# r-barnes/richdem

Hardware: AMD Instinct MI355X
Metric: Mcells/s Priority-Flood fill, 40k x 40k f32 DEM (higher is better)
Workload: dtype f32; 1 GPU; 40000x40000 float32 fractal value-noise DEM G(seed=3), FillDepressions<D8>, HBM-resident; cells=1600000000, basins=10332798, boruvka_rounds=9, pair_records=39443163, jump_passes=1, parallelism=1 GPU

## Files before the change

include/rdgpu.h:

```cpp
#ifndef RDGPU_H_
#define RDGPU_H_

#include <stdint.h>

#ifdef __cplusplus
extern "C" {
#endif

#define RDGPU_OK 0
#define RDGPU_ERR_HIP 1
#define RDGPU_ERR_ARG 2
#define RDGPU_ERR_UNSUPPORTED 3
#define RDGPU_ERR_CAPACITY 4

const char *rdgpu_last_error(void);
const char *rdgpu_version(void);
int rdgpu_device_count(int *count);
int rdgpu_set_device(int device_id);
int rdgpu_release_workspace(void);

int rdgpu_fill_u8(uint8_t *dem, int width, int height, int topology);
int rdgpu_fill_i16(int16_t *dem, int width, int height, int topology);
int rdgpu_fill_u16(uint16_t *dem, int width, int height, int topology);
int rdgpu_fill_i32(int32_t *dem, int width, int height, int topology);
// ... 124 lines not shown
  int rdgpu_watersheds_##SUF(T *dem, T nodata, int width, int height, int topology, int alter, int32_t *labels);      \
  int rdgpu_watersheds_dev_##SUF(T *d_dem, T nodata, int width, int height, int topology, int alter, int32_t *d_labels, void *hip_stream);
RDGPU_DECL_WS(u8, uint8_t)
RDGPU_DECL_WS(i16, int16_t)
RDGPU_DECL_WS(u16, uint16_t)
RDGPU_DECL_WS(i32, int32_t)
RDGPU_DECL_WS(u32, uint32_t)
RDGPU_DECL_WS(f32, float)
RDGPU_DECL_WS(i8, int8_t)
RDGPU_DECL_WS(f64, double)
RDGPU_DECL_WS(i64, int64_t)
RDGPU_DECL_WS(u64, uint64_t)
#undef RDGPU_DECL_WS

typedef struct rdgpu_fill_stats {
  uint64_t cells;
  uint64_t basins;
  uint32_t rounds;
  uint32_t jump_passes;
  uint64_t scan_tiles;
  uint32_t tile_cells;
  uint32_t edge_records;
  uint32_t host_syncs;
  uint32_t reserved;
} rdgpu_fill_stats;
int rdgpu_fill_get_stats(rdgpu_fill_stats *out);

typedef struct rdgpu_fill_shard rdgpu_fill_shard;
int rdgpu_fill_shard_begin_u8(uint8_t *d_rows, int width, int rows, int topology, int open_top, int open_bottom, void *hip_stream, rdgpu_fill_shard **out);
int rdgpu_fill_shard_begin_i16(int16_t *d_rows, int width, int rows, int topology, int open_top, int open_bottom, void *hip_stream, rdgpu_fill_shard **out);
int rdgpu_fill_shard_begin_u16(uint16_t *d_rows, int width, int rows, int topology, int open_top, int open_bottom, void *hip_stream, rdgpu_fill_shard **out);
int rdgpu_fill_shard_begin_i32(int32_t *d_rows, int width, int rows, int topology, int open_top, int open_bottom, void *hip_stream, rdgpu_fill_shard **out);
int rdgpu_fill_shard_begin_u32(uint32_t *d_rows, int width, int rows, int topology, int open_top, int open_bottom, void *hip_stream, rdgpu_fill_shard **out);
int rdgpu_fill_shard_begin_f32(float *d_rows, int width, int rows, int topology, int open_top, int open_bottom, void *hip_stream, rdgpu_fill_shard **out);
int rdgpu_fill_shard_begin_i8(int8_t *d_rows, int width, int rows, int topology, int open_top, int open_bottom, void *hip_stream, rdgpu_fill_shard **out);
int rdgpu_fill_shard_edge_count(rdgpu_fill_shard *shard, uint32_t *n_edges);
int rdgpu_fill_shard_export(rdgpu_fill_shard *shard, uint32_t *top_keys, uint32_t *bottom_keys, uint32_t *edges);
int rdgpu_fill_shard_finish(rdgpu_fill_shard *shard, const uint32_t *levels);
int rdgpu_fill_shard_free(rdgpu_fill_shard *shard);
int rdgpu_fill_graph_solve(int nshards, int width, int topology, const uint32_t *keys, const uint32_t *edges,
                           const uint64_t *edge_offsets, uint32_t *levels);
int rdgpu_fill_shard_export_dev(rdgpu_fill_shard *shard, uint32_t *d_keys, uint32_t *d_edges, uint32_t cap);
int rdgpu_fill_graph_solve_dev(int nshards, int width, int topology, const uint32_t *d_keys_all,
                               const uint32_t *d_edges_all, const uint32_t *d_counts, uint32_t cap,
                               uint32_t *d_levels_all, void *hip_stream);
int rdgpu_fill_shard_finish_dev(rdgpu_fill_shard *shard, const uint32_t *d_levels);
int rdgpu_fill_multi_u8(uint8_t *dem, int width, int height, int topology, const int *devices, int ndevices);
// ... 457 lines not shown
```

richdem_amd/_lib.py:

```python
from __future__ import annotations

import ctypes
import os
import subprocess

_HERE = os.path.dirname(os.path.abspath(__file__))
_LIB = None


class RdgpuError(RuntimeError):
    """Raised when a C-ABI call returns non-zero (mirrors the reference's std::runtime_error)."""


def lib_path() -> str:
    return os.environ.get("RDGPU_LIB") or os.path.join(_HERE, "librdgpu.so")


def build(force: bool = False) -> str:
    args = ["make", "-C", os.path.join(_HERE, "csrc"), "-j8"]
    if force:
        subprocess.check_call(args + ["clean"], stdout=subprocess.DEVNULL)
    subprocess.check_call(args, stdout=subprocess.DEVNULL)
    return lib_path()


class rdgpu_fill_stats(ctypes.Structure):
    _fields_ = [
        ("cells", ctypes.c_uint64),
        ("basins", ctypes.c_uint64),
        ("rounds", ctypes.c_uint32),
        ("jump_passes", ctypes.c_uint32),
        ("scan_tiles", ctypes.c_uint64),
        ("tile_cells", ctypes.c_uint32),
        ("edge_records", ctypes.c_uint32),
        ("host_syncs", ctypes.c_uint32),
        ("reserved", ctypes.c_uint32),
    ]


def lib() -> ctypes.CDLL:
    global _LIB
    if _LIB is None:
        p = lib_path()
        if not os.path.exists(p):
            raise RdgpuError(
                f"{p} is missing: the HIP extension is not built (run richdem_amd.build() / "
                "python -c 'import __graft_entry__ as g; g.build()').  There is no CPU fallback."
            )
        try:
            import torch
        except ImportError:
            pass
        L = ctypes.CDLL(p)
        L.rdgpu_last_error.restype = ctypes.c_char_p
        L.rdgpu_version.restype = ctypes.c_char_p
        L.rdgpu_profile_name.restype = ctypes.c_char_p
        _LIB = L
    return _LIB


def check(rc: int, what: str = "") -> None:
    if rc != 0:
        msg = lib().rdgpu_last_error().decode(errors="replace")
        err = RdgpuError(f"{what}: {msg} (code {rc})" if what else f"{msg} (code {rc})")
        err.code = rc
        raise err


def fill_stats() -> dict:
    st = rdgpu_fill_stats()
    check(lib().rdgpu_fill_get_stats(ctypes.byref(st)), "rdgpu_fill_get_stats")
    return {"cells": st.cells, "basins": st.basins, "rounds": st.rounds, "jump_passes": st.jump_passes,
            "scan_tiles": st.scan_tiles, "tile_cells": st.tile_cells, "edge_records": st.edge_records,
            "host_syncs": st.host_syncs}


def profile_enable(on: bool = True) -> None:
    lib().rdgpu_profile_enable(1 if on else 0)


def profile_collect() -> None:
    check(lib().rdgpu_profile_collect(), "rdgpu_profile_collect")


def profile_reset() -> None:
    check(lib().rdgpu_profile_reset(), "rdgpu_profile_reset")


def profile_totals() -> dict:
    L = lib()
    profile_collect()
    out = {}
    i = 0
    while True:
        nm = L.rdgpu_profile_name(i)
        if nm is None:
            break
# ... 7 lines not shown
```

richdem_amd/csrc/fill.hip:

```cpp
#include "common.hpp"
#include "fill_shared.hpp"

#include <algorithm>
#include <cstdlib>
#include <vector>

struct rdgpu_fill_shard;

namespace rdgpu {

constexpr int TW = 64;
constexpr int TH = 32;
constexpr int LW = TW + 2;
constexpr int LH = TH + 2;
constexpr uint32_t OUTP = 0xFFFFFFFFu;
constexpr uint32_t CLOSED = 0x80000000u;
constexpr uint32_t NO_TID = 0xFFFFFFFFu;

static thread_local rdgpu_fill_stats g_stats;

constexpr int DW = 64, DH = 64, DLW = DW + 2, DLH = DH + 2;
constexpr uint32_t LAB_PEND = 0x80000000u;
constexpr uint16_t LTERM_BASE = 0xF000u;

// ... 1694 lines not shown
  check_fill_args(dem, w, h, topology);
  const size_t bytes = (size_t)w * h * sizeof(T);
  T *d = Workspace::get().buf<T>("host.dem", (size_t)w * h);
  RD_HIP(hipMemcpy(d, dem, bytes, hipMemcpyHostToDevice));
  fill_max_dep_device<T>(d, w, h, topology, max_dep, nullptr);
  RD_HIP(hipStreamSynchronize(nullptr));
  RD_HIP(hipMemcpy(dem, d, bytes, hipMemcpyDeviceToHost));
}

constexpr int FSTRIPES = 32, FSTRIDE = 16;
struct FusedBuf {
  uint16_t *lab16;
  uint32_t *G;
  uint32_t *tile_base, *tile_count;
  unsigned long long *counters;
  uint32_t gcap, rcap, smask;
  uint32_t *overflow;
  uint32_t *edgeK = nullptr;
  uint16_t *edgeS = nullptr;
  uint16_t *edgeR = nullptr;
};

__global__ __launch_bounds__(64) void k_stripe_offsets(const unsigned long long *__restrict__ counters, uint32_t nstripes,
                                                       uint32_t *pitoff, uint32_t *out) {
  const uint32_t s = threadIdx.x;
  const unsigned long long c = s < nstripes ? counters[s * FSTRIDE] : 0ull;
  const uint32_t pits = (uint32_t)c, nodes = (uint32_t)(c >> 32);
  uint32_t incl = pits, tot = nodes, mx = nodes;
#pragma unroll
  for (int o = 1; o < 64; o <<= 1) {
    const uint32_t v = __shfl_up(incl, o, 64);
    if ((int)s >= o) incl += v;
    tot += __shfl_xor(tot, o, 64);
    mx = max(mx, (uint32_t)__shfl_xor(mx, o, 64));
  }
  if (s < nstripes) pitoff[s] = incl - pits;
  if (s == 63) { out[0] = incl; out[1] = tot; out[2] = mx; }
}

template <class T, int TOPO, bool VEC, bool OUTLETS = false, bool CUT = false>
__global__ __launch_bounds__(NTHR) void k_descent16(const T *__restrict__ z, FusedBuf fo, int w, int h,
                                                    uint32_t tilesX, uint32_t ntiles, const uint8_t *__restrict__ outlet = nullptr,
                                                    const uint8_t *__restrict__ skip = nullptr,
                                                    const uint32_t *__restrict__ tlist = nullptr, int open_top = 0,
                                                    int open_bottom = 0) {
  __shared__ uint32_t sk[DLH * DLW];
  constexpr int LPD = DW + 2;
  __shared__ uint16_t lp[DH * LPD];
  __shared__ uint32_t wtot[NTHR / 64];
  __shared__ uint32_t pbase, rbase, fits_s;
  const uint32_t t = (OUTLETS && tlist) ? tlist[blockIdx.x] : xcd_tile(blockIdx.x, ntiles);
  if (t >= ntiles) return;
  const int x0 = (int)(t % tilesX) * DW, y0 = (int)(t / tilesX) * DH;
  if (OUTLETS && skip && skip[t]) {
    if (threadIdx.x == 0) { fo.tile_base[t] = 0; fo.tile_count[t] = 1; }
    if (skip[t] == 1) {
      const int lx_ = threadIdx.x & (DW - 1), gx_ = x0 + lx_;
      for (int ly_ = threadIdx.x >> 6; ly_ < DH; ly_ += NTHR / 64)
        if (gx_ < w && y0 + ly_ < h) fo.lab16[(size_t)(y0 + ly_) * w + gx_] = 0;
    }
    return;
  }
  const bool inner = !OUTLETS && x0 >= 1 && y0 >= 1 && x0 + DW <= w - 1 && y0 + DH <= h - 1;
  {
    constexpr int NQ = DLH * (DW / 4), QPT = (NQ + NTHR - 1) / NTHR;
    Quad<T> zq[QPT];
    if (y0 >= 1 && y0 + DH < h && x0 + DW <= w) {
#pragma unroll
// ... 22 lines not shown
        const int gx = x0 + 4 * q, gy = y0 - 1 + ly;
        okq[r] = i < NQ && gy >= 0 && gy < h && gx < w;
        if (okq[r]) zq[r] = load_quad<T, VEC>(z + (size_t)gy * w, gx, w, T());
      }
#pragma unroll
      for (int r = 0; r < QPT; r++) keys_after_loads(zq[r]);
#pragma unroll
      for (int r = 0; r < QPT; r++) {
        const int i = threadIdx.x + r * NTHR;
        if (i >= NQ) continue;
        const int ly = i / (DW / 4), q = i - ly * (DW / 4);
        const int o = ly * DLW + 1 + 4 * q;
#pragma unroll
        for (int e = 0; e < 4; e++) sk[o + e] = (okq[r] && x0 + 4 * q + e < w) ? key32_fast<T>(zq[r].v[e]) : 0xFFFFFFFFu;
      }
    }
    for (int i = threadIdx.x; i < 2 * DLH; i += NTHR) {
      const int ly = i >> 1, lxh = (i & 1) ? DLW - 1 : 0;
      const int gx = x0 - 1 + lxh, gy = y0 - 1 + ly;
      uint32_t kk = 0xFFFFFFFFu;
      if (gx >= 0 && gx < w && gy >= 0 && gy < h) kk = key32_fast<T>(z[(size_t)gy * w + gx]);
      sk[ly * DLW + lxh] = kk;
    }
  }
  __syncthreads();
  const int wave_s = __builtin_amdgcn_readfirstlane((int)(threadIdx.x >> 6));
  const int lx = threadIdx.x & (DW - 1), ly0 = wave_s * (DH / 4);
  const int gx = x0 + lx;
  constexpr int RPT = DH / 4;
  static_assert(RPT == 16, "four code words of four bytes, 16-bit row masks");
  uint16_t *const slot16 = reinterpret_cast<uint16_t *>(sk);
  const uint32_t selfb0 = (uint32_t)((ly0 * LPD + lx) * 2);
  uint32_t p[RPT];
  uint32_t codes[RPT / 4] = {0, 0, 0, 0};
  uint32_t rootmask = 0, pitmask = 0, outmask = 0;
  {
    constexpr uint32_t WT0 = 0u | (1u << 16) | (1u << 24) | (1u << 27), WT1 = 2u | (2u << 16) | (1u << 25) | (1u << 27),
                       WT2 = 4u | (3u << 16) | (1u << 26) | (1u << 27);
    constexpr uint32_t WM0 = (uint32_t)(2 * LPD) | (4u << 16) | (1u << 24), WM2 = (uint32_t)(2 * LPD + 4) | (5u << 16) | (1u << 26);
    constexpr uint32_t BADD = (uint32_t)(4 * LPD) + (5u << 16) + ((1u << 29) - (1u << 27));
    const bool colin = gx < w, colborder = (gx == 0) | (gx == w - 1);
    const uint32_t cmcol = lx == 0 ? (1u << 24) : lx == DW - 1 ? (1u << 26) : 0u;
    uint32_t ta, tb, tc, tm, tW, ma, mb, mc, mm3, mW;
    auto triple = [&](int r, uint32_t &a, uint32_t &b, uint32_t &c, uint32_t &m, uint32_t &W) {
      a = sk[r * DLW + lx];
      b = sk[r * DLW + lx + 1];
      c = sk[r * DLW + lx + 2];
      if (TOPO == 8) {
        m = min(min(a, b), c);
        W = a == m ? WT0 : b == m ? WT1 : WT2;
      } else {
        m = b;
        W = WT1;
      }
    };
    triple(ly0, ta, tb, tc, tm, tW);
    triple(ly0 + 1, ma, mb, mc, mm3, mW);
// ... 9 lines not shown
      const uint32_t bk = min(min(tm, mm), bm);
      const bool isT = tm == bk, isM = mm == bk;
      const uint32_t wM = midfirst ? WM0 : WM2, wB = bW + BADD, wMB = isM ? wM : wB;
      const uint32_t W = isT ? tW : wMB;
      const bool drains = (bk < kc) | ((bk == kc) & (isT | (isM & midfirst)));
      uint32_t cm = cmcol;
      if (j == 0 && ly0 == 0) cm |= 1u << 27;
      if (j == RPT - 1 && ly0 == DH - RPT) cm |= 1u << 29;
      const bool outside = (W & cm) != 0u;
      const uint32_t self = selfb0 + (uint32_t)(j * LPD * 2);
      const bool incell = INNER || (colin & (gy < h));
      bool border = !INNER && (colborder | (gy == 0) | (gy == h - 1));
      bool stays = !drains;
      if (CUT && !INNER) {
        const bool cutrow = ((gy == 0) & (open_top != 0)) | ((gy == h - 1) & (open_bottom != 0));
        border = colborder | ((gy == 0) & !open_top) | ((gy == h - 1) & !open_bottom);
        stays |= cutrow;
      }
      if (OUTLETS) border |= incell && outlet[(size_t)gy * w + gx] != 0;
      const bool selfp = !incell | border | stays | outside;
      const uint32_t rel = selfp ? (uint32_t)(2 * LPD + 2) : (W & 0xFFFFu);
      p[j] = rel + (self - (uint32_t)(2 * LPD + 2));
      *reinterpret_cast<uint16_t *>(reinterpret_cast<char *>(lp) + self) = (uint16_t)p[j];
      const uint32_t cexit = (W >> 16) & 15u, cin = stays ? 0u : cexit;
      const uint32_t code = border ? 9u : cin;
      codes[j >> 2] |= code << (8 * (j & 3));
      bool root = incell & selfp;
      if (OUTLETS) {
        const bool outroot = root & border;
        outmask |= (outroot ? 1u : 0u) << j;
        root &= !outroot;
      }
      rootmask |= (root ? 1u : 0u) << j;
      pitmask |= ((root & !border & stays) ? 1u : 0u) << j;
      ta = ma; tb = mb; tc = mc; tm = mm3; tW = mW;
      ma = ba; mb = bb; mc = bc; mm3 = bm; mW = bW;
    }
    };
    if (inner) classify(std::true_type());
    else classify(std::false_type());
    (void)ta; (void)tb; (void)tc;
  }
  asm volatile("" : "+v"(rootmask), "+v"(pitmask), "+v"(outmask), "+v"(codes[0]), "+v"(codes[1]), "+v"(codes[2]), "+v"(codes[3]));
  if (fo.edgeK && threadIdx.x < 2 * DH) {
    const int side = threadIdx.x >> 6, lye = threadIdx.x & (DH - 1), lxe = side ? DW - 1 : 0;
    fo.edgeK[((size_t)t * 2 + side) * DH + lye] = sk[(lye + 1) * DLW + lxe + 1];
  }
  __syncthreads();
  {
    const char *const lpb = reinterpret_cast<const char *>(lp);
    uint32_t gact = (1u << (RPT / 4)) - 1u;
    constexpr int BLIND = 2;
    for (int it = 0; it < BLIND; it++) {
      asm volatile("" ::: "memory");
#pragma unroll
      for (int g = 0; g < RPT / 4; g++) {
        uint32_t qv[4], rv[4];
#pragma unroll
        for (int e = 0; e < 4; e++) { qv[e] = *reinterpret_cast<const uint16_t *>(lpb + p[4 * g + e]); asm("" : "+v"(qv[e])); }
#pragma unroll
        for (int e = 0; e < 4; e++) { rv[e] = *reinterpret_cast<const uint16_t *>(lpb + qv[e]); asm("" : "+v"(rv[e])); }
#pragma unroll
        for (int e = 0; e < 4; e++) {
          const int j = 4 * g + e;
          p[j] = rv[e];
          *reinterpret_cast<uint16_t *>(reinterpret_cast<char *>(lp) + selfb0 + (uint32_t)(j * LPD * 2)) = (uint16_t)rv[e];
        }
      }
    }
    for (int it = 0; gact != 0u && it < DW * DH; it++) {
      asm volatile("" ::: "memory");
// ... 18 lines not shown
    }
  }
  const uint32_t mine = ((uint32_t)__popc(rootmask) << 16) | (uint32_t)__popc(pitmask);
  uint32_t incl = mine;
#pragma unroll
  for (int o = 1; o < 64; o <<= 1) {
    const uint32_t v = __shfl_up(incl, o, 64);
    if ((threadIdx.x & 63) >= o) incl += v;
  }
  if ((threadIdx.x & 63) == 63) wtot[threadIdx.x >> 6] = incl;
  __syncthreads();
  if (threadIdx.x == 0) {
    const uint32_t nr = (wtot[0] >> 16) + (wtot[1] >> 16) + (wtot[2] >> 16) + (wtot[3] >> 16) + (OUTLETS ? 1u : 0u);
    const uint32_t np = (wtot[0] & 0xFFFFu) + (wtot[1] & 0xFFFFu) + (wtot[2] & 0xFFFFu) + (wtot[3] & 0xFFFFu);
    const uint32_t st = t & fo.smask;
    const unsigned long long old = atomicAdd(&fo.counters[st * FSTRIDE], ((unsigned long long)nr << 32) | np);
    const uint32_t rl = (uint32_t)(old >> 32);
    pbase = (uint32_t)old;
    rbase = st * fo.rcap + rl;
    fo.tile_base[t] = rbase;
    fo.tile_count[t] = nr;
    fits_s = (unsigned long long)rl + nr <= fo.rcap ? 1u : 0u;
    if (!fits_s) *fo.overflow = 1;
  }
  {
    uint32_t pre = incl - mine;
    for (int k = 0; k < wave_s; k++) pre += wtot[k];
    uint32_t slot = (pre >> 16) + (OUTLETS ? 1u : 0u);
    if (OUTLETS)
      for (uint32_t m = outmask; m; m &= m - 1)
        *reinterpret_cast<uint16_t *>(reinterpret_cast<char *>(slot16) + selfb0 + (uint32_t)((__ffs((int)m) - 1) * LPD * 2)) = 0;
    for (uint32_t m = rootmask; m; m &= m - 1) {
      const int j = __ffs((int)m) - 1;
      *reinterpret_cast<uint16_t *>(reinterpret_cast<char *>(slot16) + selfb0 + (uint32_t)(j * LPD * 2)) = (uint16_t)slot;
      slot++;
    }
  }
  __syncthreads();
  const uint32_t nodes0 = rbase;
  if (fits_s != 0) {
    uint32_t pre = incl - mine;
    for (int k = 0; k < wave_s; k++) pre += wtot[k];
    uint32_t slot = (pre >> 16) + (OUTLETS ? 1u : 0u), pit = pbase + (pre & 0xFFFFu);
    if (OUTLETS && threadIdx.x == 0) fo.G[nodes0] = OUTP;
    for (uint32_t m = rootmask; m; m &= m - 1) {
      const int j = __ffs((int)m) - 1;
      const int ly = ly0 + j;
      const uint32_t cw = j < 8 ? (j < 4 ? codes[0] : codes[1]) : (j < 12 ? codes[2] : codes[3]);
      const int code = (int)(cw >> (8 * (j & 3)) & 15u);
      const int n = code <= 4 ? code - 1 : code;
      const int nr = n >= 6 ? 2 : n >= 3 ? 1 : 0, nc = n - 3 * nr;
      const uint32_t pend = LAB_PEND | ((uint32_t)(y0 + ly + nr - 1) * (uint32_t)w + (uint32_t)(x0 + lx + nc - 1));
      const uint32_t word = code == 0 ? pit++ : code == 9 ? OUTP : pend;
      fo.G[nodes0 + slot] = word;
      slot++;
    }
  }
  {
    const char *const sl = reinterpret_cast<const char *>(slot16);
    if (inner) {
#pragma unroll
      for (int j = 0; j < RPT; j++) {
        const int gy = y0 + ly0 + j;
        fo.lab16[(size_t)gy * w + gx] = *reinterpret_cast<const uint16_t *>(sl + p[j]);
      }
    } else {
#pragma unroll
      for (int j = 0; j < RPT; j++) {
        const int gy = y0 + ly0 + j;
        const uint16_t rv = *reinterpret_cast<const uint16_t *>(sl + p[j]);
        if ((gx < w) & (gy < h)) fo.lab16[(size_t)gy * w + gx] = rv;
      }
    }
    if (fo.edgeS && threadIdx.x < 2 * DH) {
      const int side = threadIdx.x >> 6, lye = threadIdx.x & (DH - 1), lxe = side ? DW - 1 : 0;
      const uint16_t v = lp[lye * LPD + lxe];
      const bool in = inner || (x0 + lxe < w && y0 + lye < h);
      fo.edgeS[((size_t)t * 2 + side) * DH + lye] = in ? *reinterpret_cast<const uint16_t *>(sl + v) : (uint16_t)0;
    }
    if (fo.edgeR && threadIdx.x >= 2 * DH) {
      static_assert(NTHR == 2 * DH + 2 * DW, "two wavefronts for the columns, two for the rows");
      const int side = (threadIdx.x >> 6) & 1, lxe = threadIdx.x & (DW - 1), lye = side ? DH - 1 : 0;
      const uint16_t v = lp[lye * LPD + lxe];
      const bool in = inner || (x0 + lxe < w && y0 + lye < h);
      fo.edgeR[((size_t)t * 2 + side) * DW + lxe] = in ? *reinterpret_cast<const uint16_t *>(sl + v) : (uint16_t)0;
    }
  }
}

__global__ __launch_bounds__(NTHR) void k_resolve_nodes(uint32_t *G, const unsigned long long *__restrict__ counters,
                                                        const uint32_t *__restrict__ pitoff, uint32_t rcap,
                                                        const uint16_t *__restrict__ lab16,
                                                        const uint32_t *__restrict__ tile_base, int w, uint32_t tilesX,
                                                        uint32_t B, uint32_t *curN, uint32_t *flag,
                                                        const uint32_t *__restrict__ tid = nullptr,
                                                        const uint16_t *__restrict__ edgeS = nullptr,
                                                        const uint16_t *__restrict__ edgeR = nullptr) {
  const uint32_t st = blockIdx.y, i = blockIdx.x * NTHR + threadIdx.x;
  if (i >= (uint32_t)(counters[st * FSTRIDE] >> 32)) return;
  const uint32_t n = st * rcap + i;
  uint32_t v = G[n], fn = n, last = 0;
  int hops = 0;
  while ((v & LAB_PEND) && v != OUTP) {
    const uint32_t cell = v & ~LAB_PEND;
    const uint32_t cx = cell % (uint32_t)w, cy = cell / (uint32_t)w;
    const uint32_t tile = (cy / DH) * tilesX + cx / DW;
    const uint32_t lx = cx % DW, ly = cy % DH;
    const uint16_t *src = lab16 + cell;
    if (edgeS) {
      if (lx == 0u || lx == (uint32_t)(DW - 1)) src = edgeS + ((size_t)tile * 2 + (lx != 0u)) * DH + ly;
      else if (ly == 0u || ly == (uint32_t)(DH - 1)) src = edgeR + ((size_t)tile * 2 + (ly != 0u)) * DW + lx;
    }
    fn = tile_base[tile] + *src;
    last = cell;
    v = __hip_atomic_load(&G[fn], __ATOMIC_RELAXED, __HIP_MEMORY_SCOPE_AGENT);
    if (++hops > (1 << 22)) { *flag = 1; break; }
  }
  if (hops > 1) __hip_atomic_store(&G[n], LAB_PEND | last, __ATOMIC_RELAXED, __HIP_MEMORY_SCOPE_AGENT);
  if (v == OUTP || (v & LAB_PEND)) { curN[n] = B | CLOSED; return; }
  const uint32_t b = v + pitoff[fn / rcap];
  curN[n] = (tid && tid[b] != NO_TID) ? (b | CLOSED) : b;
}

__global__ __launch_bounds__(NTHR) void k_mark_terminals16(const uint16_t *__restrict__ lab16, const uint32_t *__restrict__ tile_base,
                                                           const uint32_t *__restrict__ G, const uint32_t *__restrict__ pitoff,
                                                           uint32_t rcap, uint32_t *tid, int w, int h, uint32_t dtx, int open_top,
                                                           int open_bottom) {
  const int x = blockIdx.x * NTHR + threadIdx.x;
  if (x <= 0 || x >= w - 1) return;
  if (open_top) {
    const uint32_t node = tile_base[(uint32_t)(x / DW)] + lab16[x];
    tid[G[node] + pitoff[node / rcap]] = (uint32_t)x;
  }
  if (open_bottom) {
    const uint32_t node = tile_base[(uint32_t)((h - 1) / DH) * dtx + (uint32_t)(x / DW)] + lab16[(size_t)(h - 1) * w + x];
    tid[G[node] + pitoff[node / rcap]] = (uint32_t)(w + x);
// ... 116 lines not shown
    const bool in = gx < w && gy < h;
    const size_t g = in ? (size_t)gy * w + gx : 0;
    zqs[r] = load_quad<T, VEC>(z + (g - (in ? gx : 0)), in ? gx : 0, w, T());
    lqs[r] = load_quad<uint16_t, VEC>(lab16 + (g - (in ? gx : 0)), in ? gx : 0, w, (uint16_t)0);
  }
  const uint32_t base = tile_base[t], cnt = tile_count[t];
  if (curN) {
    for (uint32_t i = threadIdx.x; i < cnt; i += NTHR) sl[i] = acc[curN[base + i] & ~CLOSED];
  } else {
    for (uint32_t i = threadIdx.x; i < cnt; i += NTHR) sl[i] = lvl[base + i];
  }
  __syncthreads();
#pragma unroll
  for (int r = 0; r < DH / 16; r++) {
    const int gy = y0 + ry + 16 * r;
    if (gx >= w || gy >= h) continue;
    const size_t g = (size_t)gy * w + gx;
    Quad<T> zq = zqs[r];
    const Quad<uint16_t> lq = lqs[r];
    bool any = false;
#pragma unroll
    for (int e = 0; e < 4; e++) {
      if (gx + e >= w) continue;
      const uint32_t L = sl[lq.v[e] & (uint16_t)(DW * DH - 1)];
      if (L > Key32<T>::to(zq.v[e])) { zq.v[e] = Key32<T>::from(L); any = true; }
    }
    if (any) {
      if (VEC) {
        struct alignas(4 * sizeof(T)) AQ { T v[4]; };
        AQ a;
#pragma unroll
        for (int e = 0; e < 4; e++) a.v[e] = zq.v[e];
        *reinterpret_cast<AQ *>(z + g) = a;
      } else {
#pragma unroll
        for (int e = 0; e < 4; e++)
          if (gx + e < w) z[g + e] = zq.v[e];
      }
    }
  }
}

constexpr int NT_CAP = 1024;
static_assert(NT_CAP * 4 <= TW * TH * 2, "the node table lives in the boundary list's storage");
static_assert(TW == DW && DH % TH == 0, "a scan tile lies inside one descent tile");
constexpr uint32_t NO_TILE = 0xFFFFFFFFu;
constexpr int RING = 2 * LW + 2 * TH;

__device__ __forceinline__ void pair_spill_local(const EdgeOut &eo, unsigned long long *best, uint32_t seg, uint32_t *seg_fill,
                                                 uint32_t lo, uint32_t hi, uint32_t key) {
  const unsigned long long cl = ((unsigned long long)key << 32) | hi, ch = ((unsigned long long)key << 32) | lo;
  if (!(lo & CLOSED) && cl < best[lo]) atomicMin(&best[lo], cl);
  if (!(hi & CLOSED) && ch < best[hi]) atomicMin(&best[hi], ch);
  const uint32_t g = atomicAdd(seg_fill, 1u);
  if (g < eo.seglimit) {
    const size_t i = (size_t)seg * eo.segcap + g;
    eo.a[i] = lo; eo.b[i] = hi; eo.k[i] = key;
  } else {
    *eo.overflow = 1;
  }
}

template <class T, int TOPO, bool VEC>
__global__ __launch_bounds__(NTHR) void k_pairs16(const T *__restrict__ z, const uint16_t *__restrict__ lab16,
                                                  const uint32_t *__restrict__ curN, unsigned long long *best,
                                                  int w, int h, uint32_t B, uint32_t tilesX,
                                                  const uint32_t *__restrict__ tiles_in, uint32_t nwork,
                                                  EdgeOut eo,
                                                  const uint32_t *__restrict__ tile_base,
// ... 29 lines not shown
  if (threadIdx.x == 0) seg_fill = 0;

  Quad<T> zq[2];
  Quad<uint16_t> lq[2];
  T rz = T();
  uint32_t rl = 0, rtb = 0, rc = 0, tbC = 0, cnt = 0, rkey = 0;
  uint32_t nt[NT_CAP / NTHR];
  auto ring_y = [](int tid) { const int rk = min(tid, RING - 1); return rk < LW ? 0 : rk < 2 * LW ? LH - 1 : (rk - 2 * LW < TH ? rk - 2 * LW + 1 : rk - 2 * LW - TH + 1); };
  auto ring_x = [](int tid) { const int rk = min(tid, RING - 1); return rk < LW ? rk : rk < 2 * LW ? rk - LW : (rk - 2 * LW < TH ? 0 : LW - 1); };

  auto load_a = [&](uint32_t t, int tid) {
    const int x0 = (int)(t % tilesX) * TW, y0 = (int)(t / tilesX) * TH;
    const uint32_t dC = (uint32_t)(y0 / DH) * dtx + (uint32_t)(x0 / DW);
    tbC = tile_base[dC];
    cnt = tile_count[dC];
    {
      const int rx = ring_x(tid), ry = ring_y(tid);
      const int gx = min(max(x0 - 1 + rx, 0), w - 1), gy = min(max(y0 - 1 + ry, 0), h - 1);
      const bool col = edgeK && ry >= 1 && ry <= TH && tid < RING;
      const uint32_t dtn = (uint32_t)(gy / DH) * dtx + (uint32_t)(gx / DW);
      const size_t e = ((size_t)dtn * 2 + (rx == 0 ? 1 : 0)) * DH + (uint32_t)(gy % DH);
      const size_t g = col ? (size_t)y0 * w + x0 : (size_t)gy * w + gx;
      rtb = tile_base[dtn];
      rl = col ? (uint32_t)edgeS[e] : (uint32_t)lab16[g];
      rkey = col ? edgeK[e] : 0u;
      rz = z[g];
    }
    const size_t tile0 = (size_t)y0 * w + x0;
    const char *zt = reinterpret_cast<const char *>(z + tile0), *lt = reinterpret_cast<const char *>(lab16 + tile0);
#pragma unroll
    for (int r = 0; r < 2; r++) {
      const int i = tid + r * NTHR;
      const int ly = i / (TW / 4), q = i - ly * (TW / 4);
      const int gx = x0 + 4 * q, gy = y0 + ly;
      const bool ok = gy < h && gx < w;
      if (VEC) {
        const uint32_t cell = ok ? (uint32_t)ly * (uint32_t)w + 4u * (uint32_t)q : 0u;
        struct alignas(4 * sizeof(T)) AZ { T v[4]; };
        struct alignas(8) AL { uint16_t v[4]; };
        const AL a = *reinterpret_cast<const AL *>(lt + cell * (uint32_t)sizeof(uint16_t));
        const AZ b = *reinterpret_cast<const AZ *>(zt + cell * (uint32_t)sizeof(T));
#pragma unroll
        for (int e = 0; e < 4; e++) { lq[r].v[e] = a.v[e]; zq[r].v[e] = b.v[e]; }
      } else {
        const size_t row = ok ? (size_t)gy * w : 0;
        lq[r] = load_quad<uint16_t, false>(lab16 + row, ok ? gx : 0, w, (uint16_t)0);
        zq[r] = load_quad<T, false>(z + row, ok ? gx : 0, w, T());
// ... 25 lines not shown
    int tid = (int)threadIdx.x;
    asm volatile("" : "+v"(tid));
    const int lx = tid & (TW - 1), band = __builtin_amdgcn_readfirstlane(tid >> 6), lane = tid & 63;
    const int rly = ring_y(tid), rlx = ring_x(tid);
    const bool isring = tid < RING;
    const int x0 = (int)(t % tilesX) * TW, y0 = (int)(t / tilesX) * TH;
    const bool tabled = cnt <= (uint32_t)NT_CAP;
    ntab[tid] = nt[0];
    if (tabled && cnt > (uint32_t)NTHR) {
#pragma unroll
      for (int k = 1; k < NT_CAP / NTHR; k++) ntab[tid + k * NTHR] = nt[k];
    }
    pt_pair[tid] = ~0ull;
    pt_key[tid] = 0xFFFFFFFFu;
    static_assert(PT_SLOTS == NTHR, "one slot per thread");
    if (tid == 0) { nlist = 0; pt_n = 0; }
    __syncthreads();
    {
      uint32_t cq[2][4];
      if (tabled) {
#pragma unroll
        for (int r = 0; r < 2; r++)
#pragma unroll
          for (int e = 0; e < 4; e++) cq[r][e] = ntab[lq[r].v[e]];
      } else {
#pragma unroll
        for (int r = 0; r < 2; r++)
#pragma unroll
          for (int e = 0; e < 4; e++) cq[r][e] = curN[tbC + (uint32_t)lq[r].v[e]];
      }
      if (x0 + TW <= w && y0 + TH <= h) {
#pragma unroll
        for (int r = 0; r < 2; r++) {
          const int i = tid + r * NTHR;
          const int ly = i / (TW / 4), q = i - ly * (TW / 4);
          const int o = (ly + 1) * LW + 1 + 4 * q;
#pragma unroll
          for (int e = 0; e < 4; e++) {
            sk[o + e] = key32_fast<T>(zq[r].v[e]);
            sc[o + e] = cq[r][e];
          }
        }
      } else {
#pragma unroll
        for (int r = 0; r < 2; r++) {
          const int i = tid + r * NTHR;
          const int ly = i / (TW / 4), q = i - ly * (TW / 4);
          const int gx = x0 + 4 * q, gy = y0 + ly;
          const int o = (ly + 1) * LW + 1 + 4 * q;
#pragma unroll
          for (int e = 0; e < 4; e++) {
            const bool in = gy < h && gx + e < w;
// ... 234 lines not shown
  fo.tile_base = (uint32_t *)persistent("fused.tile_base", (size_t)dnt * 4);
  fo.tile_count = (uint32_t *)persistent("fused.tile_count", (size_t)dnt * 4);
  uint32_t *dflags = ws.buf<uint32_t>("fused.flags", 16);
  fo.counters = (unsigned long long *)persistent("fused.counters", (size_t)FSTRIPES * FSTRIDE * 8);
  uint32_t *pitoff = ws.buf<uint32_t>("fused.pitoff", FSTRIPES);
  fo.overflow = dflags + 5;
  uint32_t *curN = (uint32_t *)persistent("fused.curN", (size_t)fo.gcap * 4);
  if (!outlet) {
    fo.edgeK = ws.buf<uint32_t>("fused.edgeK", (size_t)dnt * 2 * DH);
    fo.edgeS = ws.buf<uint16_t>("fused.edgeS", (size_t)dnt * 2 * DH);
    fo.edgeR = ws.buf<uint16_t>("fused.edgeR", (size_t)dnt * 2 * DW);
  }
  RD_HIP(hipMemsetAsync(dflags, 0, 16 * sizeof(uint32_t), s));
  RD_HIP(hipMemsetAsync(fo.counters, 0, (size_t)FSTRIPES * FSTRIDE * sizeof(unsigned long long), s));
  if (outlet) {
    static const uint32_t one = 1u, outp = OUTP;
    RD_HIP(hipMemcpyAsync(reinterpret_cast<uint32_t *>(fo.counters) + 1, &one, sizeof(uint32_t), hipMemcpyHostToDevice, s));
    RD_HIP(hipMemcpyAsync(fo.G, &outp, sizeof(uint32_t), hipMemcpyHostToDevice, s));
  }
  const bool listed = outlet && skip && lists && lists->d;
  const uint32_t *dl = listed ? lists->d : nullptr, *sl_ = listed ? lists->d + lists->stride : nullptr,
                 *fl = listed ? lists->d + 2 * (size_t)lists->stride : nullptr;
  if (listed && lists->n[0] == 0) return true;
  with_flag(vec, [&](auto V) {
    auto descent = [&](auto OUTLETS, auto CUT) {
      RD_LAUNCH("fill.descent", (k_descent16<T, TOPO, V, OUTLETS, CUT>), dim3(listed ? lists->n[0] : xcd_grid(dnt)), dim3(NTHR), 0, s,
                (const T *)d_z, fo, w, h, dtx, dnt, outlet, skip, dl, open_top, open_bottom);
    };
    if (outlet) descent(std::true_type(), std::false_type());
    else if (sharded) descent(std::false_type(), std::true_type());
    else descent(std::false_type(), std::false_type());
  });
  RD_LAUNCH("fill.stripe_offsets", k_stripe_offsets, dim3(1), dim3(64), 0, s, (const unsigned long long *)fo.counters, nstripes, pitoff,
            dflags + 8);
  RD_HIP(hipMemcpyAsync(hw, dflags + 4, 8 * sizeof(uint32_t), hipMemcpyDeviceToHost, s));
  RD_HIP(hipStreamSynchronize(s));
  g_stats.host_syncs++;
  if (hw[1] != 0) { if (getenv("RDGPU_FILL_DEBUG")) fprintf(stderr, "fill_fused: node table overflow (nstripes %u rcap %u)\n", nstripes, fo.rcap); return false; }
  const uint32_t B = hw[4], NNmax = hw[6];
  g_stats.basins = B;
  if (sharded) {
    *keep = FillBuffers();
    keep->B = B;
    if (B == 0) { keep->trivial = true; return true; }
  }
  if (B == 0) return true;
  const dim3 ngrid(cdiv(std::max(NNmax, 1u), NTHR), nstripes);
  uint32_t *tid = nullptr;
  if (sharded) {
    tid = alloc->get<uint32_t>("fill.tid", (size_t)B + 1);
    RD_HIP(hipMemsetAsync(tid, 0xFF, ((size_t)B + 1) * sizeof(uint32_t), s));
    RD_LAUNCH("fill.mark_terminals", k_mark_terminals16, dim3(cdiv(w, NTHR)), dim3(NTHR), 0, s, (const uint16_t *)fo.lab16,
              (const uint32_t *)fo.tile_base, (const uint32_t *)fo.G, (const uint32_t *)pitoff, fo.rcap, tid, w, h, dtx, open_top,
              open_bottom);
  }
  RD_LAUNCH("fill.resolve_nodes", k_resolve_nodes, ngrid, dim3(NTHR), 0, s, fo.G, (const unsigned long long *)fo.counters,
            (const uint32_t *)pitoff, fo.rcap, (const uint16_t *)fo.lab16, (const uint32_t *)fo.tile_base, w, dtx, B, curN, dflags,
            (const uint32_t *)tid, (const uint16_t *)fo.edgeS, (const uint16_t *)fo.edgeR);
  g_stats.jump_passes = 1;
  uint32_t *cur = sharded ? alloc->get<uint32_t>("fill.cur", (size_t)B + 1) : ws.buf<uint32_t>("fill.cur", (size_t)B + 1);
  uint32_t *acc = sharded ? alloc->get<uint32_t>("fill.acc", (size_t)B + 1) : ws.buf<uint32_t>("fill.acc", (size_t)B + 1);
  unsigned long long *best = ws.buf<unsigned long long>("fill.best", (size_t)B + 1);
  unsigned long long *link = ws.buf<unsigned long long>("fill.link", (size_t)B + 1);
  uint32_t *rootsA = ws.buf<uint32_t>("fill.rootsA", B);
  uint32_t *rootsB = ws.buf<uint32_t>("fill.rootsB", B);
  RD_HIP(hipMemsetAsync(dflags + 2, 0, sizeof(uint32_t), s));
  RD_LAUNCH("fill.init_tables", k_init_tables, dim3(cdiv((uint64_t)B + 1, NTHR)), dim3(NTHR), 0, s, cur, acc, link, rootsA,
            dflags + 2, (const uint32_t *)tid, B);
  uint32_t nroots0 = B;
  if (sharded) {
// ... 117 lines not shown
      if (live == 0) break;
      if (live >= last_live || rdone >= MAXR) throw Error(RDGPU_ERR_HIP, "rdgpu_fill: contraction made no progress (internal error)");
      last_live = live;
      if (!env_batch) batch = 4;
    }
  }
  g_stats.rounds += rounds_run;
  RD_LAUNCH("fill.settle_basins", k_settle_basins, dim3(cdiv(B, NTHR)), dim3(NTHR), 0, s, cur, acc, link, B, 1 << 14, dflags);
  if (sharded) {
    uint32_t *lvl = fo.G;
    RD_LAUNCH("fill.node_levels", k_node_levels, ngrid, dim3(NTHR), 0, s, (const uint32_t *)curN, (const uint32_t *)acc,
              (const unsigned long long *)fo.counters, fo.rcap, lvl);
    uint32_t *nodeW = alloc->get<uint32_t>("fused.nodeW", fo.gcap);
    RD_LAUNCH("fill.node_watersheds", k_node_watersheds, ngrid, dim3(NTHR), 0, s, (const uint32_t *)curN, (const uint32_t *)cur,
              (const uint32_t *)tid, (const unsigned long long *)fo.counters, fo.rcap, B, nodeW);
    keep->compact = true;
    keep->cur = cur; keep->acc = acc; keep->tid = tid;
    keep->lab16 = fo.lab16; keep->tile_base = fo.tile_base; keep->tile_count = fo.tile_count;
    keep->curN = curN; keep->lvl = lvl; keep->nodeW = nodeW; keep->counters = fo.counters;
    keep->rcap = fo.rcap; keep->nstripes = nstripes; keep->nnmax = NNmax;
    return true;
  }
  if (listed && lists->n[2] == 0) return true;
  with_flag(vec, [&](auto V) {
    RD_LAUNCH("fill.finalize", (k_finalize16<T, V>), dim3(listed ? lists->n[2] : xcd_grid(dnt)), dim3(NTHR), 0, s, d_z,
              (const uint16_t *)fo.lab16, (const uint32_t *)nullptr, (const uint32_t *)fo.tile_base, (const uint32_t *)fo.tile_count, w,
              h, dtx, dnt, skip, fl, (const uint32_t *)curN, (const uint32_t *)acc);
  });
  return true;
}

template <class T>
static void fill_device(T *d_z, int w, int h, int topology, hipStream_t s) {
  check_fill_args(d_z, w, h, topology);
  if (topology == 8 ? fill_fused<T, 8>(d_z, w, h, s) : fill_fused<T, 4>(d_z, w, h, s)) return;
  FillBuffers fb;
  BufAlloc ws_alloc{false, nullptr};
  if (topology == 8) fill_local_phase<T, 8>(d_z, w, h, 0, 0, ws_alloc, fb, s);
  else fill_local_phase<T, 4>(d_z, w, h, 0, 0, ws_alloc, fb, s);
  fill_finalize<T>(d_z, w, h, fb, s);
}

template <class T>
static void fill_outlets_device(T *d_z, const uint8_t *d_outlet, const uint8_t *d_skip, int w, int h, hipStream_t s,
                                const SparseLists *lists = nullptr) {
  check_fill_args(d_z, w, h, 8);
  if (!d_outlet) throw Error(RDGPU_ERR_ARG, "rdgpu_fill_outlets: null outlet mask");
  if (w <= 2 || h <= 2) return;
  if (fill_fused<T, 8>(d_z, w, h, s, d_outlet, d_skip, lists)) return;
  FillBuffers fb;
  BufAlloc ws_alloc{false, nullptr};
// ... 517 lines not shown
```

Before: 110,000 Mcells/s.

## Dissolve single-cell pits into their lowest neighbour during descent

Within the descent kernel, pits whose lowest neighbour lies inside the tile and does not drain back to them are relinked to that neighbour. They are flagged in the 16-bit label with a direction code and are no longer created as basins. Finalize raises these cells to the maximum of the basin level and their neighbour's elevation. This shrinks the basin graph that the Boruvka rounds and pair-record scans must process. The cost is extra branches and shared-memory work in descent, an extra global read per flagged cell in finalize, and label masking in the downstream kernels. It is on by default and can be turned off with an environment variable.

```diff
diff --git a/include/rdgpu.h b/include/rdgpu.h
--- a/include/rdgpu.h
+++ b/include/rdgpu.h
@@ -170,7 +170,7 @@
   uint32_t tile_cells;
   uint32_t edge_records;
   uint32_t host_syncs;
-  uint32_t reserved;
+  uint32_t dissolved_pits;
 } rdgpu_fill_stats;
 int rdgpu_fill_get_stats(rdgpu_fill_stats *out);
 
diff --git a/richdem_amd/_lib.py b/richdem_amd/_lib.py
--- a/richdem_amd/_lib.py
+++ b/richdem_amd/_lib.py
@@ -34,7 +34,7 @@
         ("tile_cells", ctypes.c_uint32),
         ("edge_records", ctypes.c_uint32),
         ("host_syncs", ctypes.c_uint32),
-        ("reserved", ctypes.c_uint32),
+        ("dissolved_pits", ctypes.c_uint32),
     ]
 
 
@@ -72,7 +72,7 @@
     check(lib().rdgpu_fill_get_stats(ctypes.byref(st)), "rdgpu_fill_get_stats")
     return {"cells": st.cells, "basins": st.basins, "rounds": st.rounds, "jump_passes": st.jump_passes,
             "scan_tiles": st.scan_tiles, "tile_cells": st.tile_cells, "edge_records": st.edge_records,
-            "host_syncs": st.host_syncs}
+            "host_syncs": st.host_syncs, "dissolved_pits": st.dissolved_pits}
 
 
 def profile_enable(on: bool = True) -> None:
diff --git a/richdem_amd/csrc/fill.hip b/richdem_amd/csrc/fill.hip
--- a/richdem_amd/csrc/fill.hip
+++ b/richdem_amd/csrc/fill.hip
@@ -1740,20 +1740,24 @@
 };
 
 __global__ __launch_bounds__(64) void k_stripe_offsets(const unsigned long long *__restrict__ counters, uint32_t nstripes,
-                                                       uint32_t *pitoff, uint32_t *out) {
+                                                       uint32_t *pitoff, uint32_t *out, uint32_t *forest_max) {
   const uint32_t s = threadIdx.x;
   const unsigned long long c = s < nstripes ? counters[s * FSTRIDE] : 0ull;
   const uint32_t pits = (uint32_t)c, nodes = (uint32_t)(c >> 32);
   uint32_t incl = pits, tot = nodes, mx = nodes;
+  uint32_t dis = s < nstripes ? (uint32_t)counters[s * FSTRIDE + 1] : 0u;
+  uint32_t mxd = nodes + dis;
 #pragma unroll
   for (int o = 1; o < 64; o <<= 1) {
     const uint32_t v = __shfl_up(incl, o, 64);
     if ((int)s >= o) incl += v;
     tot += __shfl_xor(tot, o, 64);
     mx = max(mx, (uint32_t)__shfl_xor(mx, o, 64));
+    dis += __shfl_xor(dis, o, 64);
+    mxd = max(mxd, (uint32_t)__shfl_xor(mxd, o, 64));
   }
   if (s < nstripes) pitoff[s] = incl - pits;
-  if (s == 63) { out[0] = incl; out[1] = tot; out[2] = mx; }
+  if (s == 63) { out[0] = incl; out[1] = tot; out[2] = mx; out[3] = dis; *forest_max = mxd; }
 }
 
 template <class T, int TOPO, bool VEC, bool OUTLETS = false, bool CUT = false>
@@ -1761,7 +1765,10 @@
                                                     uint32_t tilesX, uint32_t ntiles, const uint8_t *__restrict__ outlet = nullptr,
                                                     const uint8_t *__restrict__ skip = nullptr,
                                                     const uint32_t *__restrict__ tlist = nullptr, int open_top = 0,
-                                                    int open_bottom = 0) {
+                                                    int open_bottom = 0, int dissolve = 0) {
+  constexpr bool DIS_OK = !OUTLETS && !CUT;
+  const bool dis = DIS_OK && dissolve != 0;
+  __shared__ uint32_t dcnt;
   __shared__ uint32_t sk[DLH * DLW];
   constexpr int LPD = DW + 2;
   __shared__ uint16_t lp[DH * LPD];
@@ -1830,6 +1837,7 @@
       if (gx >= 0 && gx < w && gy >= 0 && gy < h) kk = key32_fast<T>(z[(size_t)gy * w + gx]);
       sk[ly * DLW + lxh] = kk;
     }
+    if (DIS_OK && threadIdx.x == 0) dcnt = 0;
   }
   __syncthreads();
   const int wave_s = __builtin_amdgcn_readfirstlane((int)(threadIdx.x >> 6));
@@ -1840,7 +1848,7 @@
   uint16_t *const slot16 = reinterpret_cast<uint16_t *>(sk);
   const uint32_t selfb0 = (uint32_t)((ly0 * LPD + lx) * 2);
   uint32_t p[RPT];
-  uint32_t codes[RPT / 4] = {0, 0, 0, 0};
+  uint32_t codesLo = 0, codesHi = 0;
   uint32_t rootmask = 0, pitmask = 0, outmask = 0;
   {
     constexpr uint32_t WT0 = 0u | (1u << 16) | (1u << 24) | (1u << 27), WT1 = 2u | (2u << 16) | (1u << 25) | (1u << 27),
@@ -1896,9 +1904,10 @@
       const uint32_t rel = selfp ? (uint32_t)(2 * LPD + 2) : (W & 0xFFFFu);
       p[j] = rel + (self - (uint32_t)(2 * LPD + 2));
       *reinterpret_cast<uint16_t *>(reinterpret_cast<char *>(lp) + self) = (uint16_t)p[j];
-      const uint32_t cexit = (W >> 16) & 15u, cin = stays ? 0u : cexit;
-      const uint32_t code = border ? 9u : cin;
-      codes[j >> 2] |= code << (8 * (j & 3));
+      const uint32_t cexit = (W >> 16) & 15u;
+      const uint32_t code = border ? 9u : cexit;
+      if (j < 8) codesLo |= code << (4 * (j & 7));
+      else codesHi |= code << (4 * (j & 7));
       bool root = incell & selfp;
       if (OUTLETS) {
         const bool outroot = root & border;
@@ -1915,12 +1924,33 @@
     else classify(std::false_type());
     (void)ta; (void)tb; (void)tc;
   }
-  asm volatile("" : "+v"(rootmask), "+v"(pitmask), "+v"(outmask), "+v"(codes[0]), "+v"(codes[1]), "+v"(codes[2]), "+v"(codes[3]));
+  asm volatile("" : "+v"(rootmask), "+v"(pitmask), "+v"(outmask), "+v"(codesLo), "+v"(codesHi));
   if (fo.edgeK && threadIdx.x < 2 * DH) {
     const int side = threadIdx.x >> 6, lye = threadIdx.x & (DH - 1), lxe = side ? DW - 1 : 0;
     fo.edgeK[((size_t)t * 2 + side) * DH + lye] = sk[(lye + 1) * DLW + lxe + 1];
   }
   __syncthreads();
+  auto code_of = [codesLo, codesHi](int j) -> int {
+    return (int)((j < 8 ? codesLo : codesHi) >> (4 * (j & 7)) & 15u);
+  };
+  uint32_t dissmask = 0;
+  if (dis) {
+    for (uint32_t m = pitmask; m; m &= m - 1) {
+      const int j = __ffs((int)m) - 1;
+      const int code = code_of(j);
+      const int n = code <= 4 ? code - 1 : code, nr = n >= 6 ? 2 : n >= 3 ? 1 : 0, nc = n - 3 * nr;
+      const int qx = lx + nc - 1, qy = ly0 + j + nr - 1;
+      if ((unsigned)qx >= (unsigned)DW || (unsigned)qy >= (unsigned)DH) continue;
+      const uint32_t self = selfb0 + (uint32_t)(j * LPD * 2), qb = (uint32_t)((qy * LPD + qx) * 2);
+      if ((uint32_t)*reinterpret_cast<const uint16_t *>(reinterpret_cast<const char *>(lp) + qb) == self) continue;
+      *reinterpret_cast<uint16_t *>(reinterpret_cast<char *>(lp) + self) = (uint16_t)qb;
+      dissmask |= 1u << j;
+    }
+    rootmask &= ~dissmask;
+    pitmask &= ~dissmask;
+    if (dissmask) atomicAdd(&dcnt, (uint32_t)__popc(dissmask));
+    __syncthreads();
+  }
   {
     const char *const lpb = reinterpret_cast<const char *>(lp);
     uint32_t gact = (1u << (RPT / 4)) - 1u;
@@ -1985,6 +2015,7 @@
     fo.tile_count[t] = nr;
     fits_s = (unsigned long long)rl + nr <= fo.rcap ? 1u : 0u;
     if (!fits_s) *fo.overflow = 1;
+    if (DIS_OK && dis && dcnt != 0u) atomicAdd(&fo.counters[st * FSTRIDE + 1], (unsigned long long)dcnt);
   }
   {
     uint32_t pre = incl - mine;
@@ -2009,12 +2040,11 @@
     for (uint32_t m = rootmask; m; m &= m - 1) {
       const int j = __ffs((int)m) - 1;
       const int ly = ly0 + j;
-      const uint32_t cw = j < 8 ? (j < 4 ? codes[0] : codes[1]) : (j < 12 ? codes[2] : codes[3]);
-      const int code = (int)(cw >> (8 * (j & 3)) & 15u);
+      const int code = code_of(j);
       const int n = code <= 4 ? code - 1 : code;
       const int nr = n >= 6 ? 2 : n >= 3 ? 1 : 0, nc = n - 3 * nr;
       const uint32_t pend = LAB_PEND | ((uint32_t)(y0 + ly + nr - 1) * (uint32_t)w + (uint32_t)(x0 + lx + nc - 1));
-      const uint32_t word = code == 0 ? pit++ : code == 9 ? OUTP : pend;
+      const uint32_t word = (pitmask >> j & 1u) ? pit++ : code == 9 ? OUTP : pend;
       fo.G[nodes0 + slot] = word;
       slot++;
     }
@@ -2035,6 +2065,13 @@
         if ((gx < w) & (gy < h)) fo.lab16[(size_t)gy * w + gx] = rv;
       }
     }
+    if (DIS_OK)
+      for (uint32_t m = dissmask; m; m &= m - 1) {
+        const int j = __ffs((int)m) - 1;
+        const uint32_t root = *reinterpret_cast<const uint16_t *>(reinterpret_cast<const char *>(lp) + selfb0 + (uint32_t)(j * LPD * 2));
+        const uint32_t slot = *reinterpret_cast<const uint16_t *>(sl + root);
+        fo.lab16[(size_t)(y0 + ly0 + j) * w + gx] = (uint16_t)(slot | ((8u | (uint32_t)(code_of(j) - 1)) << 12));
+      }
     if (fo.edgeS && threadIdx.x < 2 * DH) {
       const int side = threadIdx.x >> 6, lye = threadIdx.x & (DH - 1), lxe = side ? DW - 1 : 0;
       const uint16_t v = lp[lye * LPD + lxe];
@@ -2074,7 +2111,7 @@
       if (lx == 0u || lx == (uint32_t)(DW - 1)) src = edgeS + ((size_t)tile * 2 + (lx != 0u)) * DH + ly;
       else if (ly == 0u || ly == (uint32_t)(DH - 1)) src = edgeR + ((size_t)tile * 2 + (ly != 0u)) * DW + lx;
     }
-    fn = tile_base[tile] + *src;
+    fn = tile_base[tile] + (*src & (uint16_t)(DW * DH - 1));
     last = cell;
     v = __hip_atomic_load(&G[fn], __ATOMIC_RELAXED, __HIP_MEMORY_SCOPE_AGENT);
     if (++hops > (1 << 22)) { *flag = 1; break; }
@@ -2237,7 +2274,14 @@
 #pragma unroll
     for (int e = 0; e < 4; e++) {
       if (gx + e >= w) continue;
-      const uint32_t L = sl[lq.v[e] & (uint16_t)(DW * DH - 1)];
+      const uint32_t lab = lq.v[e];
+      uint32_t L = sl[lab & (uint32_t)(DW * DH - 1)];
+      if (lab & 0x8000u) {
+        const int d = (int)(lab >> 12) & 7, n = d < 4 ? d : d + 1, nr = n >= 6 ? 2 : n >= 3 ? 1 : 0, nc = n - 3 * nr;
+        const T zn = z[(size_t)(gy + nr - 1) * w + (size_t)(gx + e + nc - 1)];
+        const uint32_t kq = Key32<T>::to(zn);
+        L = kq > L ? kq : L;
+      }
       if (L > Key32<T>::to(zq.v[e])) { zq.v[e] = Key32<T>::from(L); any = true; }
     }
     if (any) {
@@ -2260,6 +2304,7 @@
 static_assert(NT_CAP * 4 <= TW * TH * 2, "the node table lives in the boundary list's storage");
 static_assert(TW == DW && DH % TH == 0, "a scan tile lies inside one descent tile");
 constexpr uint32_t NO_TILE = 0xFFFFFFFFu;
+constexpr uint32_t LAB16_SLOT = (uint32_t)(DW * DH - 1);
 constexpr int RING = 2 * LW + 2 * TH;
 
 __device__ __forceinline__ void pair_spill_local(const EdgeOut &eo, unsigned long long *best, uint32_t seg, uint32_t *seg_fill,
@@ -2335,7 +2380,7 @@
       const size_t e = ((size_t)dtn * 2 + (rx == 0 ? 1 : 0)) * DH + (uint32_t)(gy % DH);
       const size_t g = col ? (size_t)y0 * w + x0 : (size_t)gy * w + gx;
       rtb = tile_base[dtn];
-      rl = col ? (uint32_t)edgeS[e] : (uint32_t)lab16[g];
+      rl = col ? (uint32_t)edgeS[e] : (uint32_t)lab16[g] & LAB16_SLOT;
       rkey = col ? edgeK[e] : 0u;
       rz = z[g];
     }
@@ -2407,12 +2452,12 @@
 #pragma unroll
         for (int r = 0; r < 2; r++)
 #pragma unroll
-          for (int e = 0; e < 4; e++) cq[r][e] = ntab[lq[r].v[e]];
+          for (int e = 0; e < 4; e++) cq[r][e] = ntab[lq[r].v[e] & LAB16_SLOT];
       } else {
 #pragma unroll
         for (int r = 0; r < 2; r++)
 #pragma unroll
-          for (int e = 0; e < 4; e++) cq[r][e] = curN[tbC + (uint32_t)lq[r].v[e]];
+          for (int e = 0; e < 4; e++) cq[r][e] = curN[tbC + ((uint32_t)lq[r].v[e] & LAB16_SLOT)];
       }
       if (x0 + TW <= w && y0 + TH <= h) {
 #pragma unroll
@@ -2693,30 +2738,51 @@
   const uint32_t *dl = listed ? lists->d : nullptr, *sl_ = listed ? lists->d + lists->stride : nullptr,
                  *fl = listed ? lists->d + 2 * (size_t)lists->stride : nullptr;
   if (listed && lists->n[0] == 0) return true;
+  const char *env_dis = getenv("RDGPU_FILL_DISSOLVE");
+  const int dissolve = (!outlet && !sharded && !(env_dis && env_dis[0] == '0')) ? 1 : 0;
   with_flag(vec, [&](auto V) {
     auto descent = [&](auto OUTLETS, auto CUT) {
       RD_LAUNCH("fill.descent", (k_descent16<T, TOPO, V, OUTLETS, CUT>), dim3(listed ? lists->n[0] : xcd_grid(dnt)), dim3(NTHR), 0, s,
-                (const T *)d_z, fo, w, h, dtx, dnt, outlet, skip, dl, open_top, open_bottom);
+                (const T *)d_z, fo, w, h, dtx, dnt, outlet, skip, dl, open_top, open_bottom, dissolve);
     };
     if (outlet) descent(std::true_type(), std::false_type());
     else if (sharded) descent(std::false_type(), std::true_type());
     else descent(std::false_type(), std::false_type());
   });
   RD_LAUNCH("fill.stripe_offsets", k_stripe_offsets, dim3(1), dim3(64), 0, s, (const unsigned long long *)fo.counters, nstripes, pitoff,
-            dflags + 8);
+            dflags + 8, dflags + 6);
   RD_HIP(hipMemcpyAsync(hw, dflags + 4, 8 * sizeof(uint32_t), hipMemcpyDeviceToHost, s));
   RD_HIP(hipStreamSynchronize(s));
   g_stats.host_syncs++;
-  if (hw[1] != 0) { if (getenv("RDGPU_FILL_DEBUG")) fprintf(stderr, "fill_fused: node table overflow (nstripes %u rcap %u)\n", nstripes, fo.rcap); return false; }
+  if (hw[1] != 0 || hw[2] > fo.rcap) { if (getenv("RDGPU_FILL_DEBUG")) fprintf(stderr, "fill_fused: node table overflow (nstripes %u rcap %u)\n", nstripes, fo.rcap); return false; }
   const uint32_t B = hw[4], NNmax = hw[6];
-  g_stats.basins = B;
+  const uint32_t ndis = hw[7];
+  g_stats.basins = (uint64_t)B + ndis;
+  g_stats.dissolved_pits = ndis;
   if (sharded) {
     *keep = FillBuffers();
     keep->B = B;
     if (B == 0) { keep->trivial = true; return true; }
   }
-  if (B == 0) return true;
+  if (B == 0 && ndis == 0) return true;
   const dim3 ngrid(cdiv(std::max(NNmax, 1u), NTHR), nstripes);
+  auto finalize = [&](const uint32_t *curN_, const uint32_t *acc_) {
+    with_flag(vec, [&](auto V) {
+      RD_LAUNCH("fill.finalize", (k_finalize16<T, V>), dim3(listed ? lists->n[2] : xcd_grid(dnt)), dim3(NTHR), 0, s, d_z,
+                (const uint16_t *)fo.lab16, (const uint32_t *)nullptr, (const uint32_t *)fo.tile_base, (const uint32_t *)fo.tile_count, w,
+                h, dtx, dnt, skip, fl, curN_, acc_);
+    });
+  };
+  if (B == 0) {
+    uint32_t *acc0 = ws.buf<uint32_t>("fill.acc", 1);
+    RD_HIP(hipMemsetAsync(acc0, 0, sizeof(uint32_t), s));
+    RD_LAUNCH("fill.resolve_nodes", k_resolve_nodes, ngrid, dim3(NTHR), 0, s, fo.G, (const unsigned long long *)fo.counters,
+              (const uint32_t *)pitoff, fo.rcap, (const uint16_t *)fo.lab16, (const uint32_t *)fo.tile_base, w, dtx, B, curN, dflags,
+              (const uint32_t *)nullptr, (const uint16_t *)fo.edgeS, (const uint16_t *)fo.edgeR);
+    g_stats.jump_passes = 1;
+    finalize(curN, acc0);
+    return true;
+  }
   uint32_t *tid = nullptr;
   if (sharded) {
     tid = alloc->get<uint32_t>("fill.tid", (size_t)B + 1);
@@ -2880,11 +2946,7 @@
     return true;
   }
   if (listed && lists->n[2] == 0) return true;
-  with_flag(vec, [&](auto V) {
-    RD_LAUNCH("fill.finalize", (k_finalize16<T, V>), dim3(listed ? lists->n[2] : xcd_grid(dnt)), dim3(NTHR), 0, s, d_z,
-              (const uint16_t *)fo.lab16, (const uint32_t *)nullptr, (const uint32_t *)fo.tile_base, (const uint32_t *)fo.tile_count, w,
-              h, dtx, dnt, skip, fl, (const uint32_t *)curN, (const uint32_t *)acc);
-  });
+  finalize((const uint32_t *)curN, (const uint32_t *)acc);
   return true;
 }
 
```

Measured after the change: 116,900 Mcells/s (median of 6 runs). +6.3%, better.
